# plume-sig/zk-nullifier-sig

Measured on AMD Instinct MI355X. Metric: PLUME verifies/sec (secp256k1 V1) at batch=2^20 per GPU, higher is better.
Workload: dtype u32; 1 GPU; BASELINE.json configs[1]/metric: batch 2^20 per GPU, PLUME V1 verify (secp256k1 + SHA-256), 32-byte messages, 1/16 corrupted, inputs resident in HBM; Fp arithmetic on 9x29-bit limbs through chains of v_mad_u64_u32 (32x32+64); items_per_gpu=1048576, parallelism=shard x1, no collective on the data path, world_size=1

## Files before the change

__graft_entry__.py:

```python
import os
import subprocess
import sys
from pathlib import Path

ROOT = Path(__file__).resolve().parent
os.environ.setdefault("HSA_ENABLE_IPC_MODE_LEGACY", "0")
os.environ.setdefault("GPU_MAX_HW_QUEUES", "8")
if str(ROOT) not in sys.path:
    sys.path.insert(0, str(ROOT))


def build() -> None:
    env = dict(os.environ, PYTORCH_ROCM_ARCH="gfx950")
    subprocess.check_call(["make", "-j2", "-C", str(ROOT / "zk-nullifier-sig_amd" / "csrc")], env=env)
    subprocess.check_call(["make", "-C", str(ROOT / "oracle")])
    subprocess.check_call(["make", "-C", str(ROOT / "tests" / "devsim")])
    subprocess.check_call(["make", "-C", str(ROOT / "tests" / "devgpu")])
    import zk_nullifier_sig_amd as plume
    assert plume.library_path().exists()


def smoke() -> None:
    import numpy as np

    import zk_nullifier_sig_amd as plume
    from oracle import plume_oracle as O
    from tests import _oracle_c as OC
    from tests import synth

    eng = plume.Engine(0)
    n = 64
    for ver in (1, 2):
        b = synth.sign_inputs(n)
        got = eng.sign_batch(ver, b["msgs"], b["off"], b["sk"], b["r"])
        want = OC.sign_batch(ver, b["msgs"], b["off"], b["sk"], b["r"], nthreads=4)
        for k in got:
            assert np.array_equal(got[k], want[k]), f"sign v{ver}: {k} differs from the oracle"
        v = synth.corrupt_for_verify(ver, b, got)
        ok = eng.verify_batch(ver, v["msgs"], v["off"], v["pk"], v["nullifier"], v["c"], v["s"], v.get("r_point"), v.get("hashed_to_curve_r"))
        want_ok = OC.verify_batch(ver, v["msgs"], v["off"], v["pk"], v["nullifier"], v["c"], v["s"], v.get("r_point"), v.get("hashed_to_curve_r"), nthreads=4)
        assert np.array_equal(ok, want_ok), f"verify v{ver} differs from the oracle"
        assert list(ok) == [0 if i % 16 == 5 else 1 for i in range(n)]
        nz = (ver, b["msgs"], b["off"], got["pk"], got["nullifier"], got["s"], got["r_point"], got["hashed_to_curve_r"], got["c"])
        assert np.array_equal(eng.verify_non_zk_batch(*nz), OC.verify_non_zk_batch(*nz, nthreads=4)), f"verify_non_zk v{ver} differs from the oracle"

    class Mock:
        def fill_bytes(self, k):
            return bytes.fromhex("93b9323b629f251b8f3fc2dd11f4672c5544e8230d493eceea98a90bda789808")

    sk = plume.SecretKey.from_bytes(bytes.fromhex("519b423d715f8b581f4fa8ee59f4771a5b44c8130b4e3eacca54a56dda72b464"))
    sig = plume.PlumeSignature.sign_v1(sk, b"An example app message string", Mock(), eng)
    assert sig.c.to_bytes().hex() == "c6a7fc2c926ddbaf20731a479fb6566f2daa5514baae5223fe3b32edbce83254"
    assert sig.s.to_bytes().hex() == "e69f027d84cb6fe5f761e333d12e975fb190d163e8ea132d7de0bd6079ba28ca"
    assert sig.verify(eng)
    assert O.verify(1, sig.message, (sig.pk.x, sig.pk.y), (sig.nullifier.x, sig.nullifier.y), sig.c.value, sig.s.value,
                    (sig.v1specific.r_point.x, sig.v1specific.r_point.y), (sig.v1specific.hashed_to_curve_r.x, sig.v1specific.hashed_to_curve_r.y))
    eng.close()
    print("smoke ok:", plume.library_path())


if __name__ == "__main__":
    build() if (len(sys.argv) < 2 or sys.argv[1] == "build") else smoke()
```

zk-nullifier-sig_amd/csrc/plume_capi.hip:

```cpp
#include <hip/hip_runtime.h>

#include <sched.h>

#include <cctype>
#include <condition_variable>
#include <cstdio>
#include <cstdlib>
#include <cstring>
#include <functional>
#include <iterator>
#include <map>
#include <mutex>
#include <cerrno>
#include <sys/random.h>
#include <string>
#include <thread>
#include <tuple>
#include <initializer_list>
#include <algorithm>
#include <atomic>
#include <memory>
#include <vector>

#include "../../include/plume_hip.h"
// ... 672 lines not shown
}

struct RecoverCall {
    RecoverLaunch fn;
    int version, format;
    uint8_t *rpt, *hr, *h, *status;
};

static int verify_device(plume_ctx* ctx, int version, int mode, size_t n, const uint8_t* msgs, const uint64_t* msg_off, size_t msgs_bytes, const uint8_t* pk, const uint8_t* nul,
                         const uint8_t* c, const uint8_t* s, const uint8_t* rpt, const uint8_t* hr, uint8_t* ok, hipStream_t st,
                         const uint8_t* preflags = nullptr, bool continue_timer = false, const uint8_t* rpt33 = nullptr, const uint8_t* hr33 = nullptr,
                         const RecoverCall* rec = nullptr) {
    if (n == 0) return 0;
    if (n > ctx->chunk) return fail(PLUME_ERR_ARG, "n exceeds the chunk size (plume_set_chunk)");
    if (int rc = need_gtab(ctx)) return rc;
    const bool eq1short = verify_eq1_short(ctx, version, mode, n, rpt != nullptr && rpt33 == nullptr);
    if (eq1short) { if (int rc = need_gcomb(ctx)) return rc; }
    const size_t J = eq1short ? 4 : 3;
    if (!continue_timer) { if (int rc = ws_acquire(ctx, st)) return rc; }
    std::unique_ptr<WsHold> hold(continue_timer ? nullptr : new WsHold(ctx, st));
    const std::vector<size_t> cut = sub_batch_bounds(ctx, n);
    const size_t nsub = cut.size() - 1;
    const bool overlapped = nsub > 1;
    if (int rc = verify_workspace(ctx, n, J, cut)) return rc;
    if (overlapped) { if (int rc = pre_events(ctx, nsub)) return rc; if (int rc = pre_stream(ctx)) return rc; }
    StageTimer& t = ctx->timer;
    if (!continue_timer) t.begin(st);
    hipStream_t pre = overlapped ? ctx->pre : st;
    if (overlapped) {
        HIPCHK(hipEventRecord(ctx->pre_begin, st));
        HIPCHK(hipStreamWaitEvent(pre, ctx->pre_begin, 0));
    }
    for (size_t k = 0; k < nsub; k++) {
        const size_t lo = cut[k], cnt = cut[k + 1] - cut[k];
        VerifyArgs a;
        memset(&a, 0, sizeof a);
        a.version = version; a.mode = mode; a.n = (uint32_t)cnt; a.msgs = msgs; a.msg_off = msg_off + lo; a.msgs_bytes = msgs_bytes;
        a.pk = pk + 64 * lo; a.nul = nul + 64 * lo; a.c = c + 32 * lo; a.s = s + 32 * lo; a.rpt = rpt ? rpt + 64 * lo : nullptr; a.hr = hr ? hr + 64 * lo : nullptr; a.ok = ok ? ok + lo : nullptr;
        a.preflags = preflags ? preflags + lo : nullptr; a.rpt33 = rpt33 ? rpt33 + 33 * lo : nullptr; a.hr33 = hr33 ? hr33 + 33 * lo : nullptr;
        a.bases = ctx->bases.as<uint32_t>() + (size_t)PLUME_BASE_WORDS * J * lo; a.jobflags = ctx->jobflags.as<uint8_t>() + J * lo; a.itemflags = ctx->itemflags.as<uint8_t>() + lo;
        a.tab = ctx->tab.as<uint32_t>() + (size_t)PLUME_TAB_WORDS * J * lo; a.res = ctx->res.as<uint32_t>() + (size_t)PLUME_JAC_WORDS * 2 * lo; a.resinf = ctx->resinf.as<uint8_t>() + 2 * lo;
        a.gtab = ctx->fixed->gtab.as<uint32_t>();
        a.redo = ctx->redo.as<uint32_t>() + 2 * lo + k;
        a.digs = ctx->digs.as<int8_t>() + (size_t)PLUME_VDIG_ROWS * lo;
        if (eq1short) {
            a.eq1fall = ctx->eq1fall.as<uint8_t>() + lo; a.eq1k = ctx->eq1k.as<uint32_t>() + 8 * lo; a.gcomb = ctx->fixed->gcomb.as<uint32_t>();
            a.eq1force = ctx->eq1_short == 2 ? 1 : 0;
        }
        if (k == 0) ctx->redo_counters.clear();
        ctx->redo_counters.push_back(2 * lo + k);
        const bool two_roles = cnt <= ctx->ingest_split_max;
        a.msm_pair = (!eq1short && cnt <= ctx->msm_pair_max) ? 1 : 0;
        a.scalars_in_ingest = two_roles && ctx->split_scalars ? 1 : 0;
        launch_verify_ingest(a, pre, two_roles); if (!overlapped) t.stage(a.scalars_in_ingest ? "verify_ingest_h2c+scalars" : "verify_ingest_h2c", st);
        if (!a.scalars_in_ingest) { launch_verify_scalars(a, pre); if (!overlapped) t.stage("verify_scalars", st); }
        table_stage(ctx, a.tab, a.bases, a.jobflags, J * cnt, 3 * cnt, pre); if (!overlapped) t.stage("tables", st);
        if (overlapped) {
            HIPCHK(hipEventRecord(ctx->pre_ready[k], pre));
            HIPCHK(hipStreamWaitEvent(st, ctx->pre_ready[k], 0));
        }
        ctx->last_msm_kernel = verify_msm_kernel_name(a);
        if (k == 0) ctx->last_msm_sampled = false;
        if (t.on && !overlapped && k == 0) {
            if (ctx->clk.ensure(16)) return PLUME_ERR_HIP;
            HIPCHK(hipMemsetAsync(ctx->clk.p, 0, 16, st));
            a.clk = ctx->clk.as<unsigned long long>();
            ctx->last_msm_sampled = true;
        }
        launch_verify_msm(a, st); if (!overlapped) t.stage("verify_msm", st);
        if (version == 2 && mode == PLUME_MODE_VERIFY) { launch_normalize(a.res, a.resinf, 2 * cnt, st); if (!overlapped) t.stage("to_affine", st); }
        if (rec) {
            const size_t P = recover_width(rec->format);
            RecoverArgs ra;
            memset(&ra, 0, sizeof ra);
            ra.version = rec->version; ra.format = rec->format; ra.n = a.n; ra.pk = a.pk; ra.nul = a.nul; ra.c = a.c;
            ra.itemflags = a.itemflags; ra.jobflags = a.jobflags; ra.tab = a.tab; ra.res = a.res; ra.resinf = a.resinf;
            ra.rpt = rec->rpt ? rec->rpt + P * lo : nullptr; ra.hr = rec->hr ? rec->hr + P * lo : nullptr; ra.h = rec->h ? rec->h + P * lo : nullptr;
            ra.status = rec->status ? rec->status + lo : nullptr;
            rec->fn(ra, st); if (!overlapped) t.stage("recover_finalize", st);
        } else {
            launch_verify_finalize(a, st); if (!overlapped) t.stage("verify_finalize", st);
        }
    }
    if (overlapped) t.stage("verify_overlapped", st);
    HIPCHK(hipGetLastError());
    return hold ? hold->release() : 0;
}

static int sign_device(plume_ctx* ctx, int version, size_t n, const uint8_t* msgs, const uint64_t* msg_off, size_t msgs_bytes, const uint8_t* sk, const uint8_t* r,
                       const uint8_t* pk_in, uint8_t* pk, uint8_t* nul, uint8_t* c, uint8_t* s, uint8_t* rpt, uint8_t* hr, uint8_t* status, uint8_t* h_out,
                       hipStream_t st, bool out33 = false, const uint8_t* aux = nullptr, SignNonceLaunch nonce_fn = nullptr) {
    if (n == 0) return 0;
    if (n > ctx->chunk) return fail(PLUME_ERR_ARG, "n exceeds the chunk size (plume_set_chunk)");
    if (int rc = need_sign_tables(ctx)) return rc;
    const bool selfcheck = ctx->sign_selfcheck != 0;
    const SignReleaseLaunch release_fn = selfcheck ? g_sign_release.load() : nullptr;
    if (selfcheck && !release_fn) return fail(PLUME_ERR_ARG, "the signer's self-check is on but its release kernel is not part of this build");
    const bool sc_eq1short = selfcheck && verify_eq1_short(ctx, version, PLUME_MODE_NON_ZK, n, true);
    if (selfcheck) { if (int rc = need_fixed(ctx, true, sc_eq1short, false)) return rc; }
    if (int rc = ws_acquire(ctx, st)) return rc;
    WsHold hold(ctx, st);
    const std::vector<size_t> cut = sub_batch_bounds(ctx, n);
    constexpr size_t kStageBytes = 4 * 64 + 2 * 32 + 2;
    if (selfcheck && (verify_workspace(ctx, n, sc_eq1short ? 4 : 3, cut) || ctx->scstage.ensure(kStageBytes * n) || (ctx->timer.on && ctx->clk.ensure(16)))) return PLUME_ERR_HIP;
    uint8_t* const stg = ctx->scstage.as<uint8_t>();
    uint8_t *const g_pk = stg, *const g_nul = stg + 64 * n, *const g_rpt = stg + 128 * n, *const g_hr = stg + 192 * n, *const g_c = stg + 256 * n, *const g_s = stg + 288 * n,
            *const g_status = stg + 320 * n, *const g_ok = stg + 321 * n;
    struct StageWipe {
        plume_ctx* ctx; size_t bytes; hipStream_t st;
        ~StageWipe() { if (bytes) (void)hipMemsetAsync(ctx->scstage.p, 0, bytes, st); }
    } stage_wipe{ctx, selfcheck ? kStageBytes * n : 0, st};
    uint8_t *const u_pk = pk, *const u_nul = nul, *const u_c = c, *const u_s = s, *const u_rpt = rpt, *const u_hr = hr, *const u_status = status;
    const bool u_out33 = out33;
    if (selfcheck) { pk = g_pk; nul = g_nul; c = g_c; s = g_s; rpt = g_rpt; hr = g_hr; status = g_status; out33 = false; }
    const size_t nsub = cut.size() - 1;
    const bool overlapped = nsub > 1;
    size_t scr_bytes = 0;
    constexpr size_t SK = PLUME_SIGN_K;
    for (size_t k = 0; k < nsub; k++) scr_bytes = std::max(scr_bytes, table_stage_scratch(ctx, SK * (cut[k + 1] - cut[k]), 0));
    if (ctx->bases.ensure((size_t)PLUME_BASE_WORDS * 4 * SK * n) || ctx->jobflags.ensure(SK * n) || ctx->itemflags.ensure(n) || ctx->tab.ensure((size_t)PLUME_TAB_WORDS * 4 * SK * n) ||
        ctx->tabscr.ensure(scr_bytes) ||
// ... 1441 lines not shown
```

zk-nullifier-sig_amd/csrc/plume_ec.h:

```cpp
#pragma once
#include "plume_field.h"

#if !defined(__HIP_DEVICE_COMPILE__) && defined(PLUME_FE_CHECK)
namespace plume { inline unsigned long& fallback_counter() { static unsigned long c = 0; return c; } }
#define PLUME_COUNT_FALLBACK() (++plume::fallback_counter())
#else
#define PLUME_COUNT_FALLBACK() ((void)0)
#endif

namespace plume {

struct jac {
    fe x, y, z;
    uint32_t inf;
};

PLUME_HD fe fe_beta() { return fe_set(0x7AE96A2Bu, 0x657C0710u, 0x6E64479Eu, 0xAC3434E9u, 0x9CF04975u, 0x12F58995u, 0xC1396C28u, 0x719501EEu); }
PLUME_HD fe fe_gx() { return fe_set(0x79BE667Eu, 0xF9DCBBACu, 0x55A06295u, 0xCE870B07u, 0x029BFCDBu, 0x2DCE28D9u, 0x59F2815Bu, 0x16F81798u); }
PLUME_HD fe fe_gy() { return fe_set(0x483ADA77u, 0x26A3C465u, 0x5DA4FBFCu, 0x0E1108A8u, 0xFD17B448u, 0xA6855419u, 0x9C47D08Fu, 0xFB10D4B8u); }

PLUME_HD fe fe_off_x() { return fe_set(0xBE71E685u, 0x6986BD54u, 0xA5797708u, 0x9EF9F753u, 0x1397E48Bu, 0x08AA9EB1u, 0x128983CAu, 0x1D5B099Bu); }
PLUME_HD fe fe_off_y() { return fe_set(0x15AE5773u, 0x1FAF9233u, 0xF016B8C3u, 0x84D627FDu, 0x8CF7C500u, 0x22EAB6A1u, 0x27C3954Bu, 0x8A01ED04u); }
PLUME_HD fe fe_off_c128_x() { return fe_set(0x8141C548u, 0xF0861E56u, 0xAE562CECu, 0x00E54F8Bu, 0x7535C0B1u, 0x943A12D3u, 0x469080E1u, 0xA23EEBF9u); }
PLUME_HD fe fe_off_c128_y() { return fe_set(0xE429892Au, 0x9AB04F55u, 0xF3E86FE7u, 0xE225348Fu, 0xEF934040u, 0xDC585E87u, 0x1A3CC5BEu, 0x78194203u); }
// ... 206 lines not shown
        if (pos + PLUME_GW_BYTES < PLUME_NDIG) {
            PLUME_UNROLL for (int b = 0; b < PLUME_GW_BYTES; b++) dig[(uint32_t)(pos + b) * stride] = (int8_t)(uint8_t)((mag >> (8 * b)) & 0xFF);
            dig[(uint32_t)(pos + PLUME_GW_BYTES) * stride] = sgn;
        } else if (pos + 1 < PLUME_NDIG) {
            dig[(uint32_t)pos * stride] = (int8_t)(uint8_t)(mag & 0xFF);
            dig[(uint32_t)(pos + 1) * stride] = (int8_t)(uint8_t)(((mag >> 8) & 0x7F) | (sgn ? 0x80 : 0));
        } else {
            dig[(uint32_t)pos * stride] = (int8_t)(uint8_t)((mag & 0x3F) | (sgn ? 0x40 : 0));
        }
    }
}
#define PLUME_NPOS 65
#define PLUME_NPOS64 33
#define PLUME_NPOS66 34
#ifndef PLUME_SIGN_K
#define PLUME_SIGN_K 2
#endif
#define PLUME_SIGN_BITS (128 / PLUME_SIGN_K)
#define PLUME_NPOSK (PLUME_SIGN_BITS / 2 + 1)
static_assert(PLUME_SIGN_K == 2 || PLUME_SIGN_K == 4, "pieces of 64 or 32 bits (whole words of the GLV halves)");
PLUME_HD uint32_t eisd_entry_table(int ta, int tb) {
    static const uint16_t T[64] = {0x240, 0x343, 0x44F, 0x144, 0x261, 0x366, 0x469, 0x167, 0x28D, 0x38C, 0x492, 0x10B, 0x222, 0x328, 0x02A, 0x125,
                                   0x240, 0x343, 0x44F, 0x144, 0x261, 0x366, 0x469, 0x167, 0x28D, 0x38C, 0x011, 0x10B, 0x222, 0x328, 0x02A, 0x125,
                                   0x240, 0x343, 0x44F, 0x144, 0x261, 0x366, 0x469, 0x167, 0x28D, 0x38C, 0x011, 0x10B, 0x222, 0x328, 0x02A, 0x125,
                                   0x240, 0x343, 0x44F, 0x144, 0x261, 0x366, 0x469, 0x167, 0x28D, 0x38C, 0x011, 0x10B, 0x222, 0x328, 0x02A, 0x125};
    const uint32_t idx = (((uint32_t)ta & 3u) << 2) | ((uint32_t)tb & 3u) | (ta < 0 ? 16u : 0u) | (tb < 0 ? 32u : 0u);
    return T[idx];
}
PLUME_HD uint32_t eisd_entry(int ta, int tb) {
    const uint32_t i = (((uint32_t)ta & 3u) << 2) | ((uint32_t)tb & 3u);
    const uint64_t CLO = 0x5C98D3A4C123C60ull, CHI = 0x2A902ull, D0 = 0x2491246DB492ull, D1 = 0x21A31A31A31Aull;
    uint32_t code = (uint32_t)((i < 12u ? CLO >> (5u * i) : CHI >> (5u * (i - 12u))) & 31u);
    uint32_t d0 = (uint32_t)(D0 >> (3u * i)) & 7u, d1 = (uint32_t)(D1 >> (3u * i)) & 7u;
    if (i == 10u && (ta < 0 || tb < 0)) { code = 17u; d0 = 0u; d1 = 0u; }
    return code | (d0 << 5) | (d1 << 8);
}
template <int NP, int NW>
PLUME_HD bool eisd_store(int8_t* dig, uint32_t stride, const uint32_t (&am)[NW], bool aneg, const uint32_t (&bm)[NW], bool bneg, bool flip) {
    const int sa = (aneg != flip) ? -1 : 1, sb = (bneg != flip) ? -1 : 1;
    int ca = 0, cb = 0;
    PLUME_UNROLL for (int i = 0; i < NP; i++) {
        const int w = (2 * i) >> 5, sh = (2 * i) & 31;
        const int cha = w < NW ? (int)((am[w < NW ? w : 0] >> sh) & 3u) : 0, chb = w < NW ? (int)((bm[w < NW ? w : 0] >> sh) & 3u) : 0;
        const int ta = sa * cha + ca, tb = sb * chb + cb;
        const uint32_t e = eisd_entry(ta, tb);
        dig[(uint32_t)i * stride] = (int8_t)(e & 31u);
        ca = (ta - ((int)((e >> 5) & 7u) - 2)) >> 2;
        cb = (tb - ((int)((e >> 8) & 7u) - 2)) >> 2;
    }
    return ca == 0 && cb == 0;
}
PLUME_HD void eisd_store_glv(int8_t* dig, uint32_t stride, const glv_half& h1, const glv_half& h2, bool flip) {
    (void)eisd_store<PLUME_NPOS, 4>(dig, stride, h1.m, h1.neg != 0, h2.m, h2.neg != 0, flip);
}

#define PLUME_TAB_ENTRIES 3
#define PLUME_FE_W PLUME_FE_WORDS
#define PLUME_JAC_WORDS (3 * PLUME_FE_WORDS)
#define PLUME_TAB_ENTRY_WORDS 32
#define PLUME_TAB_WORDS (PLUME_TAB_ENTRIES * PLUME_TAB_ENTRY_WORDS)

PLUME_HD void ld_tab_xy(fe& x, fe& y, const uint32_t* e, bool lambda_half) {
    const uint32_t* xs = lambda_half ? e + 16 : e;
    PLUME_UNROLL for (int i = 0; i < 8; i++) { x.v[i] = xs[i]; y.v[i] = e[8 + i]; }
    x.v[8] = lambda_half ? e[26] : e[24];
    y.v[8] = e[25];
}
template <int ROWS>
PLUME_HD void ld_tab_xy_scan(fe& x, fe& y, const uint32_t* tab, int ad, bool lambda_half) {
    ld_tab_xy(x, y, tab, lambda_half);
    PLUME_NOUNROLL for (int e = 1; e < ROWS; e++) {
        fe rx, ry;
        ld_tab_xy(rx, ry, tab + (size_t)e * PLUME_TAB_ENTRY_WORDS, lambda_half);
        const bool take = ad == e + 1;
        fe_cmov(x, rx, take); fe_cmov(y, ry, take);
    }
}
PLUME_HD void st_tab_entry(uint32_t* e, const fe& x, const fe& y, const fe& bx) {
    PLUME_UNROLL for (int i = 0; i < 8; i++) { e[i] = x.v[i]; e[8 + i] = y.v[i]; e[16 + i] = bx.v[i]; }
    e[24] = x.v[8]; e[25] = y.v[8]; e[26] = bx.v[8]; e[27] = 0;
    e[28] = 0; e[29] = 0; e[30] = 0; e[31] = 0;
}
PLUME_HD void ld_fe(fe& r, const uint32_t* p) { PLUME_UNROLL for (int i = 0; i < PLUME_FE_W; i++) r.v[i] = p[i]; }
PLUME_HD void st_fe(uint32_t* p, const fe& a) { PLUME_UNROLL for (int i = 0; i < PLUME_FE_W; i++) p[i] = a.v[i]; }
PLUME_HD void ld_fe_soa(fe& r, const uint32_t* base, size_t stride, size_t j) { PLUME_UNROLL for (int i = 0; i < PLUME_FE_W; i++) r.v[i] = base[(size_t)i * stride + j]; }
PLUME_HD void st_fe_soa(uint32_t* base, size_t stride, size_t j, const fe& a) { PLUME_UNROLL for (int i = 0; i < PLUME_FE_W; i++) base[(size_t)i * stride + j] = a.v[i]; }
PLUME_HD void ld_jac_soa(jac& p, const uint32_t* base, size_t stride, size_t j) {
    ld_fe_soa(p.x, base, stride, j); ld_fe_soa(p.y, base + PLUME_FE_W * stride, stride, j); ld_fe_soa(p.z, base + 2 * PLUME_FE_W * stride, stride, j);
}
PLUME_HD void st_jac_soa(uint32_t* base, size_t stride, size_t j, const jac& p) {
    st_fe_soa(base, stride, j, p.x); st_fe_soa(base + PLUME_FE_W * stride, stride, j, p.y); st_fe_soa(base + 2 * PLUME_FE_W * stride, stride, j, p.z);
}
#define PLUME_BASE_WORDS 28
struct alignas(16) quad32 { uint32_t a, b, c, d; };
PLUME_HD void st_base(uint32_t* bases, size_t job, const jac& p) {
    quad32* q = reinterpret_cast<quad32*>(bases + job * PLUME_BASE_WORDS);
    q[0] = quad32{p.x.v[0], p.x.v[1], p.x.v[2], p.x.v[3]}; q[1] = quad32{p.x.v[4], p.x.v[5], p.x.v[6], p.x.v[7]};
    q[2] = quad32{p.x.v[8], p.y.v[0], p.y.v[1], p.y.v[2]}; q[3] = quad32{p.y.v[3], p.y.v[4], p.y.v[5], p.y.v[6]};
    q[4] = quad32{p.y.v[7], p.y.v[8], p.z.v[0], p.z.v[1]}; q[5] = quad32{p.z.v[2], p.z.v[3], p.z.v[4], p.z.v[5]};
    q[6] = quad32{p.z.v[6], p.z.v[7], p.z.v[8], 0u};
}
PLUME_HD void ld_base(jac& p, const uint32_t* bases, size_t job, bool with_z) {
    const quad32* q = reinterpret_cast<const quad32*>(bases + job * PLUME_BASE_WORDS);
    const quad32 q0 = q[0], q1 = q[1], q2 = q[2], q3 = q[3], q4 = q[4];
    p.x.v[0] = q0.a; p.x.v[1] = q0.b; p.x.v[2] = q0.c; p.x.v[3] = q0.d; p.x.v[4] = q1.a; p.x.v[5] = q1.b; p.x.v[6] = q1.c; p.x.v[7] = q1.d; p.x.v[8] = q2.a;
    p.y.v[0] = q2.b; p.y.v[1] = q2.c; p.y.v[2] = q2.d; p.y.v[3] = q3.a; p.y.v[4] = q3.b; p.y.v[5] = q3.c; p.y.v[6] = q3.d; p.y.v[7] = q4.a; p.y.v[8] = q4.b;
// ... 458 lines not shown
```

zk-nullifier-sig_amd/csrc/plume_eis.h:

```cpp
#pragma once
#include "plume_ec.h"

namespace plume {

constexpr int kEisR = 5, kEisT = 3;
constexpr int32_t kEisMask = (1 << 29) - 1;

PLUME_HD double eis_fma(double a, double b, double c) { return __builtin_fma(a, b, c); }
template <int N>
PLUME_HD double eis_to_double(const int32_t (&l)[N]) {
    double d = (double)l[N - 1];
    PLUME_UNROLL for (int i = N - 2; i >= 0; i--) d = eis_fma(d, 536870912.0, (double)l[i]);
    return d;
}
template <int N>
PLUME_HD void eis_reduce(int32_t (&x0)[N], int32_t (&x1)[N], const int32_t (&y0)[N], const int32_t (&y1)[N], int32_t q0, int32_t q1) {
    int64_t c0 = 0, c1 = 0;
    PLUME_UNROLL for (int i = 0; i < N; i++) {
        const int32_t z = y0[i] - y1[i];
        c0 += (int64_t)x0[i] - (int64_t)q0 * y0[i] + (int64_t)q1 * y1[i];
        c1 += (int64_t)x1[i] - (int64_t)q0 * y1[i] - (int64_t)q1 * z;
        if (i < N - 1) { x0[i] = (int32_t)c0 & kEisMask; c0 >>= 29; x1[i] = (int32_t)c1 & kEisMask; c1 >>= 29; }
        else { x0[i] = (int32_t)c0; x1[i] = (int32_t)c1; }
    }
// ... 43 lines not shown
    PLUME_UNROLL for (int i = 0; i < N; i++) { x0[i] = x.c0[i]; x1[i] = x.c1[i]; }
}

struct eis_short {
    uint32_t t[2][3], u[2][3];
    uint32_t tneg[2], uneg[2];
    sc tau;
    bool ok;
};
template <int N>
PLUME_HD void eis_from_half(int32_t (&l)[N], const glv_half& h) {
    const uint32_t* m = h.m;
    int32_t v[5];
    v[0] = (int32_t)(m[0] & (uint32_t)kEisMask);
    v[1] = (int32_t)(((m[0] >> 29) | (m[1] << 3)) & (uint32_t)kEisMask);
    v[2] = (int32_t)(((m[1] >> 26) | (m[2] << 6)) & (uint32_t)kEisMask);
    v[3] = (int32_t)(((m[2] >> 23) | (m[3] << 9)) & (uint32_t)kEisMask);
    v[4] = (int32_t)(m[3] >> 20);
    int32_t cy = 0;
    PLUME_UNROLL for (int i = 0; i < N; i++) {
        const int32_t t = (h.neg ? -(i < 5 ? v[i] : 0) : (i < 5 ? v[i] : 0)) + cy;
        if (i < N - 1) { l[i] = t & kEisMask; cy = t >> 29; } else l[i] = t;
    }
}
template <int N>
PLUME_HD bool eis_abs66(uint32_t (&mag)[3], uint32_t& neg, const int32_t (&l)[N]) {
    neg = l[N - 1] < 0 ? 1u : 0u;
    int32_t v[N];
    int32_t cy = 0;
    PLUME_UNROLL for (int i = 0; i < N; i++) {
        const int32_t t = (neg ? -l[i] : l[i]) + cy;
        if (i < N - 1) { v[i] = t & kEisMask; cy = t >> 29; } else v[i] = t;
    }
    const uint32_t a = (uint32_t)v[0], b = (uint32_t)v[1], c = (uint32_t)v[2], d = N > 3 ? (uint32_t)v[N > 3 ? 3 : 0] : 0u;
    mag[0] = a | (b << 29);
    mag[1] = (b >> 3) | (c << 26);
    mag[2] = (c >> 6) | (d << 23);
    bool small = (mag[2] >> 2) == 0 && (N <= 3 || (d >> 9) == 0);
    PLUME_UNROLL for (int i = 4; i < N; i++) small = small && v[i] == 0;
    return small;
}

constexpr int kEisMaxSteps = 400;
PLUME_HD void eis_half_gcd(eis_short& out, const glv_half& g0, const glv_half& g1) {
    const glv_half pa = {{0x9284EB15u, 0xE86C90E4u, 0xA7D46BCDu, 0x3086D221u}, 0u}, pb = {{0x0ABFE4C3u, 0x6F547FA9u, 0x010E8828u, 0xE4437ED6u}, 1u};
    int32_t x0[kEisR], x1[kEisR], y0[kEisR], y1[kEisR];
    eis_from_half(x0, pa); eis_from_half(x1, pb);
    eis_from_half(y0, g0); eis_from_half(y1, g1);
    int32_t tx0[kEisT] = {0, 0, 0}, tx1[kEisT] = {0, 0, 0}, ty0[kEisT] = {1, 0, 0}, ty1[kEisT] = {0, 0, 0};
    double dx0 = eis_to_double(x0), dx1 = eis_to_double(x1), dy0 = eis_to_double(y0), dy1 = eis_to_double(y1);
    const double T = 340282366920938463463374607431768211456.0;
    int which = -1;
    PLUME_NOUNROLL for (int it = 0; it < kEisMaxSteps; it++) {
        if (eis_norm(dy0, dy1) < T) { which = 1; break; }
        int32_t q0, q1; int k;
        eis_quotient(q0, q1, k, dx0, dx1, dy0, dy1);
        eis_step(x0, x1, y0, y1, q0, q1, k);
        eis_step(tx0, tx1, ty0, ty1, q0, q1, k);
        dx0 = eis_to_double(x0); dx1 = eis_to_double(x1);
        if (eis_norm(dx0, dx1) < T) { which = 0; break; }
        eis_quotient(q0, q1, k, dy0, dy1, dx0, dx1);
        eis_step(y0, y1, x0, x1, q0, q1, k);
        eis_step(ty0, ty1, tx0, tx1, q0, q1, k);
        dy0 = eis_to_double(y0); dy1 = eis_to_double(y1);
    }
    const bool sel = which == 1;
    int32_t r0[kEisR], r1[kEisR], t0[kEisT], t1[kEisT];
    PLUME_UNROLL for (int i = 0; i < kEisR; i++) { r0[i] = sel ? y0[i] : x0[i]; r1[i] = sel ? y1[i] : x1[i]; }
    PLUME_UNROLL for (int i = 0; i < kEisT; i++) { t0[i] = sel ? ty0[i] : tx0[i]; t1[i] = sel ? ty1[i] : tx1[i]; }
    bool ok = which >= 0;
    uint32_t m0[3], m1[3], n0, n1;
    ok = eis_abs66(m0, n0, t0) && ok;
    ok = eis_abs66(m1, n1, t1) && ok;
    {
        sc a, b, lam, bl;
        PLUME_UNROLL for (int i = 0; i < 8; i++) { a.v[i] = i < 3 ? m0[i] : 0u; b.v[i] = i < 3 ? m1[i] : 0u; }
        const uint32_t L[8] = {0x1B23BD72u, 0xDF02967Cu, 0x20816678u, 0x122E22EAu, 0x8812645Au, 0xA5261C02u, 0xC05C30E0u, 0x5363AD4Cu};
        PLUME_UNROLL for (int i = 0; i < 8; i++) lam.v[i] = L[i];
        sc_mul(bl, b, lam);
        if (n1) sc_neg(bl, bl);
        if (n0) sc_neg(a, a);
        sc_add(out.tau, a, bl);
        ok = ok && !sc_is_zero(out.tau);
    }
    {
        t0[0] -= 1;
        int32_t cy = 0;
        PLUME_UNROLL for (int i = 0; i < kEisT; i++) { const int32_t t = t0[i] + cy; if (i < kEisT - 1) { t0[i] = t & kEisMask; cy = t >> 29; } else t0[i] = t; }
    }
    ok = eis_abs66(out.t[0], out.tneg[0], t0) && ok;
    PLUME_UNROLL for (int i = 0; i < 3; i++) out.t[1][i] = m1[i];
    out.tneg[1] = n1;
    ok = eis_abs66(out.u[0], out.uneg[0], r0) && ok;
    ok = eis_abs66(out.u[1], out.uneg[1], r1) && ok;
    out.ok = ok;
}

PLUME_HD bool eis_consistent(const eis_short& e, const sc& c) {
    const uint32_t L[8] = {0x1B23BD72u, 0xDF02967Cu, 0x20816678u, 0x122E22EAu, 0x8812645Au, 0xA5261C02u, 0xC05C30E0u, 0x5363AD4Cu};
    sc a, b, lam, bl, ups, lhs;
    PLUME_UNROLL for (int i = 0; i < 8; i++) { a.v[i] = i < 3 ? e.u[0][i] : 0u; b.v[i] = i < 3 ? e.u[1][i] : 0u; lam.v[i] = L[i]; }
    sc_mul(bl, b, lam);
    if (e.uneg[1]) sc_neg(bl, bl);
    if (e.uneg[0]) sc_neg(a, a);
    sc_add(ups, a, bl);
    sc_mul(lhs, e.tau, c);
    uint32_t d = 0;
    PLUME_UNROLL for (int i = 0; i < 8; i++) d |= lhs.v[i] ^ ups.v[i];
    return d == 0;
}

}
```

zk-nullifier-sig_amd/csrc/plume_kernels.hip:

```cpp
#include <algorithm>

#include "plume_launch.h"
#include "plume_dedup.h"

#define PLUME_MIN_WAVES 4
#define PLUME_MSM_WAVES PLUME_MIN_WAVES
#define PLUME_H2C_WAVES 3
#define PLUME_FINAL_WAVES 2
#define PLUME_NORM_WAVES 2
#define PLUME_BOUNDS __launch_bounds__(kBlock, PLUME_MIN_WAVES)
#define PLUME_FINAL_BOUNDS __launch_bounds__(kBlock, PLUME_FINAL_WAVES)
#define PLUME_NORM_BOUNDS __launch_bounds__(kBlock, PLUME_NORM_WAVES)
#define PLUME_MSM_BOUNDS __launch_bounds__(kBlock, PLUME_MSM_WAVES)
#define PLUME_H2C_BOUNDS __launch_bounds__(kBlock, PLUME_H2C_WAVES)

namespace plume {



__global__ PLUME_BOUNDS void k_fixed_bases(uint32_t* base18, uint32_t nwin, uint32_t W) {
    const uint32_t w = blockIdx.x * kBlock + threadIdx.x;
    if (w < nwin) fixed_window_base(base18 + (size_t)w * 2 * PLUME_FE_W, W * w);
}
__global__ PLUME_BOUNDS void k_fixed_table(uint32_t* rows, const uint32_t* base18, uint32_t entries, uint32_t nwin) {
    const size_t lane = (size_t)blockIdx.x * kBlock + threadIdx.x;
    if (lane < (size_t)entries * nwin) fixed_table_lane(rows, base18, entries, lane);
}

__global__ __launch_bounds__(kBlock, 4) void k_verify_scalars(VerifyArgs a) {
    const uint32_t i = blockIdx.x * kBlock + threadIdx.x;
    if (i == 0) a.redo[0] = 0;
    if (i < a.n) verify_scalars(a, i);
}

__global__ PLUME_H2C_BOUNDS void k_verify_ingest(VerifyArgs a) {
    uint32_t i = blockIdx.x * kBlock + threadIdx.x;
    if (i < a.n) verify_ingest_h2c(a, i);
}

__global__ PLUME_H2C_BOUNDS void k_verify_ingest_split(VerifyArgs a) {
    constexpr uint32_t H = kBlock / 2;
    __shared__ uint32_t s_u1[PLUME_FE_WORDS * H];
    __shared__ uint32_t s_q[3 * PLUME_FE_WORDS * H];
    __shared__ uint32_t s_fb[H];
    const uint32_t l = threadIdx.x & (H - 1);
    const bool roleB = threadIdx.x >= H;
    const uint32_t i = blockIdx.x * H + l;
    const bool live = i < a.n;
    if (a.scalars_in_ingest && blockIdx.x == 0 && threadIdx.x == H) a.redo[0] = 0;
    ingest_xch x;
    ingest_a_state st;
    if (live) {
        if (roleB) { verify_ingest_b1(a, i, x); s_fb[l] = x.fb; }
        else { verify_ingest_a1(a, i, x, st); PLUME_UNROLL for (int k = 0; k < PLUME_FE_WORDS; k++) s_u1[k * H + l] = x.u1.v[k]; }
    }
    __syncthreads();
    if (live) {
        if (roleB) {
            PLUME_UNROLL for (int k = 0; k < PLUME_FE_WORDS; k++) x.u1.v[k] = s_u1[k * H + l];
            verify_ingest_b2(x);
            PLUME_UNROLL for (int k = 0; k < PLUME_FE_WORDS; k++) { s_q[k * H + l] = x.xn.v[k]; s_q[(PLUME_FE_WORDS + k) * H + l] = x.xd.v[k]; s_q[(2 * PLUME_FE_WORDS + k) * H + l] = x.y.v[k]; }
        } else {
            x.fb = s_fb[l];
            verify_ingest_a2(a, i, x, st);
        }
    }
    __syncthreads();
    if (live && !roleB) {
        PLUME_UNROLL for (int k = 0; k < PLUME_FE_WORDS; k++) { x.xn.v[k] = s_q[k * H + l]; x.xd.v[k] = s_q[(PLUME_FE_WORDS + k) * H + l]; x.y.v[k] = s_q[(2 * PLUME_FE_WORDS + k) * H + l]; }
        verify_ingest_a3(a, i, x, st);
    } else if (live && a.scalars_in_ingest) {
        verify_scalars(a, i);
    }
}

struct WaveRowSink {
    uint4* rows;
    uint32_t** ptrs;
    bool full;
    __device__ void sync() const { __builtin_amdgcn_fence(__ATOMIC_ACQ_REL, "wavefront"); __builtin_amdgcn_wave_barrier(); }
    __device__ void operator()(uint32_t* e, const fe& x, const fe& y, const fe& bx) const {
        if (!full) { st_tab_entry(e, x, y, bx); return; }
        const uint32_t lane = threadIdx.x & 63u, sw = lane & 7u;
        uint4* mine = rows + lane * 8;
        mine[0 ^ sw] = make_uint4(x.v[0], x.v[1], x.v[2], x.v[3]);
        mine[1 ^ sw] = make_uint4(x.v[4], x.v[5], x.v[6], x.v[7]);
        mine[2 ^ sw] = make_uint4(y.v[0], y.v[1], y.v[2], y.v[3]);
        mine[3 ^ sw] = make_uint4(y.v[4], y.v[5], y.v[6], y.v[7]);
        mine[4 ^ sw] = make_uint4(bx.v[0], bx.v[1], bx.v[2], bx.v[3]);
        mine[5 ^ sw] = make_uint4(bx.v[4], bx.v[5], bx.v[6], bx.v[7]);
        mine[6 ^ sw] = make_uint4(x.v[8], y.v[8], bx.v[8], 0u);
        mine[7 ^ sw] = make_uint4(0u, 0u, 0u, 0u);
        ptrs[lane] = e;
        __builtin_amdgcn_fence(__ATOMIC_RELEASE, "wavefront");
        __builtin_amdgcn_wave_barrier();
        __builtin_amdgcn_fence(__ATOMIC_ACQUIRE, "wavefront");
        const uint32_t quad = lane & 7u;
        PLUME_UNROLL for (uint32_t q = 0; q < 8; q++) {
            const uint32_t r = (lane >> 3) + 8u * q;
            const uint4 v = rows[r * 8 + (quad ^ (r & 7u))];
            reinterpret_cast<uint4*>(ptrs[r])[quad] = v;
        }
        __builtin_amdgcn_fence(__ATOMIC_RELEASE, "wavefront");
        __builtin_amdgcn_wave_barrier();
    }
};

#define PLUME_TABPASS_WAVES_A 4
#define PLUME_TABPASS_WAVES_B 3
#define PLUME_TABINV_K 8
constexpr int kTabBlock = 128;
__global__ __launch_bounds__(kTabBlock, PLUME_TABPASS_WAVES_A) void k_tab_pass_a(const uint32_t* bases, const uint8_t* jobflags, size_t njobs, int L, uint32_t* scr, uint32_t* carry, uint8_t* guardf) {
    const size_t lane = (size_t)blockIdx.x * kTabBlock + threadIdx.x, nl = (size_t)gridDim.x * kTabBlock;
    const size_t j0 = lane * (size_t)L;
    const int cnt = j0 < njobs ? (int)((njobs - j0) < (size_t)L ? (njobs - j0) : (size_t)L) : 0;
    uint32_t* myscr = scr + (size_t)blockIdx.x * ((size_t)L * PLUME_TAB_SCR_WORDS * kTabBlock);
    fe c;
    bool g = false;
    tab_pass_a(bases, jobflags, njobs, j0, cnt, myscr, (size_t)kTabBlock, threadIdx.x, c, g);
    st_fe_soa(carry, nl, lane, c); guardf[lane] = g ? 1 : 0;
}
__global__ __launch_bounds__(kTabBlock, PLUME_TABPASS_WAVES_B) void k_tab_pass_b(uint32_t* tab, const uint32_t* bases, const uint8_t* jobflags, size_t njobs, int L, const uint32_t* scr, const uint32_t* carry,
                                                                                  const uint8_t* guardf) {
    __shared__ uint4 s_rows[kTabBlock * 8];
    __shared__ uint32_t* s_ptrs[kTabBlock];
// ... 370 lines not shown
```

zk-nullifier-sig_amd/csrc/plume_stages.h:

```cpp
#pragma once
#include "plume_h2c.h"
#include "plume_eis.h"

namespace plume {

PLUME_HD uint32_t load_affine_be(fe& x, fe& y, const uint8_t* p) {
    uint32_t wx[8], wy[8];
    words_from_be_aligned(wx, p);
    words_from_be_aligned(wy, p + 32);
    fe_from_words(x, wx);
    fe_from_words(y, wy);
    uint32_t nz = 0;
    PLUME_UNROLL for (int i = 0; i < 8; i++) nz |= wx[i] | wy[i];
    if (nz == 0) return PLUME_JOB_INF;
    if (!words_lt_p(wx) || !words_lt_p(wy)) return PLUME_JOB_INVALID;
    return affine_on_curve(x, y) ? PLUME_JOB_OK : PLUME_JOB_INVALID;
}
PLUME_HD uint32_t reload_affine_be(fe& x, fe& y, const uint8_t* p) {
    uint32_t wx[8], wy[8];
    words_from_be_aligned(wx, p);
    words_from_be_aligned(wy, p + 32);
    fe_from_words(x, wx);
    fe_from_words(y, wy);
    uint32_t nz = 0;
// ... 75 lines not shown
    const bool ok = o1 >= o0 && o1 <= msgs_bytes && o1 - o0 <= 0xFFFFFF00ull;
    len = ok ? (uint32_t)(o1 - o0) : 0u;
    if (!ok) o0 = 0;
    return ok;
}

#define PLUME_MODE_VERIFY 0
#define PLUME_MODE_NON_ZK 1
#define PLUME_ITEM_REJECT 1u
#define PLUME_ITEM_ERR 2u
struct VerifyArgs {
    int version;
    int mode;
    uint32_t n;
    const uint8_t* msgs; const uint64_t* msg_off;
    uint64_t msgs_bytes;
    const uint8_t *pk, *nul, *c, *s, *rpt, *hr;
    uint8_t* ok;
    const uint8_t* preflags;
    const uint8_t *rpt33, *hr33;
    uint32_t* bases;
    uint8_t* jobflags;
    uint8_t* itemflags;
    uint32_t* tab;
    uint32_t* res;
    uint8_t* resinf;
    const uint32_t* gtab;
    uint32_t* redo;
    int8_t* digs;
    uint8_t* eq1fall;
    uint32_t* eq1k;
    const uint32_t* gcomb;
    int msm_pair;
    int scalars_in_ingest;
    unsigned long long* clk;
    int eq1force;
};
PLUME_HD bool verify_eq1_short(const VerifyArgs& a) { return a.eq1fall != nullptr; }
PLUME_HD size_t verify_njobs(const VerifyArgs& a) { return (verify_eq1_short(a) ? 4 : 3) * (size_t)a.n; }
#define PLUME_VDIG_SET PLUME_NPOS
#define PLUME_VDIG_SETB (2 * PLUME_NPOS66)
#define PLUME_VDIG_ROWS (2 * PLUME_VDIG_SET + PLUME_VDIG_SETB)
static_assert(PLUME_VDIG_SETB >= 2 * PLUME_NDIG, "set B holds either form");
PLUME_HD uint32_t redo_file(uint32_t* redo, uint32_t task) {
#if defined(__HIP_DEVICE_COMPILE__)
    const uint32_t k = atomicAdd(redo, 1u);
#else
    const uint32_t k = redo[0]++;
#endif
    redo[1 + k] = task;
    return k;
}

PLUME_HD void verify_item_digits(int8_t* d, uint32_t n, const sc& s, const glv_half& c1, const glv_half& c2, bool long_b) {
    glv_half h1, h2;
    glv_split(h1, h2, s);
    eisd_store_glv(d, n, h1, h2, false);
    if (long_b) { booth_store_wide(d + (size_t)PLUME_VDIG_SET * n, n, h1, false); booth_store_wide(d + (size_t)(PLUME_VDIG_SET + PLUME_NDIG) * n, n, h2, false); }
    eisd_store_glv(d + (size_t)(PLUME_VDIG_SET + PLUME_VDIG_SETB) * n, n, c1, c2, true);
}
PLUME_HD void verify_scalars(const VerifyArgs& a, uint32_t i) {
    sc c, s;
    bool okc = load_scalar_be(c, a.c + 32 * (size_t)i), oks = load_scalar_be(s, a.s + 32 * (size_t)i);
    if (a.mode == PLUME_MODE_NON_ZK) { okc = sc_lt_n(c); oks = sc_lt_n(s); }
    if (!okc || !oks) { if (verify_eq1_short(a)) a.eq1fall[i] = 1; return; }
    bool lng = true;
    glv_half c1, c2;
    glv_split(c1, c2, c);
    if (verify_eq1_short(a)) {
        eis_short e;
        eis_half_gcd(e, c1, c2);
        lng = !e.ok || a.eq1force != 0 || !eis_consistent(e, c);
        if (!lng) {
            sc k;
            sc_mul(k, e.tau, s);
            PLUME_UNROLL for (int w = 0; w < 8; w++) a.eq1k[(size_t)w * a.n + i] = k.v[w];
            int8_t* b = a.digs + (size_t)PLUME_VDIG_SET * a.n + i;
            (void)eisd_store<PLUME_NPOS66, 3>(b, a.n, e.u[0], e.uneg[0] != 0, e.u[1], e.uneg[1] != 0, true);
            (void)eisd_store<PLUME_NPOS66, 3>(b + (size_t)PLUME_NPOS66 * a.n, a.n, e.t[0], e.tneg[0] != 0, e.t[1], e.tneg[1] != 0, true);
        }
        a.eq1fall[i] = lng ? 1 : 0;
    }
    verify_item_digits(a.digs + i, a.n, s, c1, c2, lng);
}

PLUME_HD void verify_ingest_h2c(const VerifyArgs& a, uint32_t i) {
    fe pkx, pky, nx, ny;
    uint32_t fpk = load_affine_be(pkx, pky, a.pk + 64 * (size_t)i);
    uint32_t fnul = load_affine_be(nx, ny, a.nul + 64 * (size_t)i);
    sc c, s;
    bool okc = load_scalar_be(c, a.c + 32 * (size_t)i), oks = load_scalar_be(s, a.s + 32 * (size_t)i);
    if (a.mode == PLUME_MODE_NON_ZK) { okc = sc_lt_n(c); oks = sc_lt_n(s); }
    uint64_t o0; uint32_t mlen;
    const bool okm = msg_span(o0, mlen, a.msg_off, i, a.msgs_bytes);
    bool bad = !okc || !oks || !okm || fpk == PLUME_JOB_INVALID || fnul == PLUME_JOB_INVALID || (a.preflags && a.preflags[i]);
    const bool err = a.mode == PLUME_MODE_NON_ZK && !bad && fpk == PLUME_JOB_INF;
    a.itemflags[i] = (uint8_t)(bad ? PLUME_ITEM_REJECT : err ? PLUME_ITEM_ERR : 0u);
    bad = bad || err;
    if (verify_eq1_short(a)) {
        fe rx, ry;
        const uint32_t fr = load_affine_be(rx, ry, a.rpt + 64 * (size_t)i);
        if (fr == PLUME_JOB_INVALID && !err) { bad = true; a.itemflags[i] = (uint8_t)PLUME_ITEM_REJECT; }
        jac p; p.inf = 0; p.z = fe_small(1); p.x = rx; p.y = ry;
        st_base(a.bases, 3 * (size_t)a.n + i, p); a.jobflags[3 * (size_t)a.n + i] = (uint8_t)(fr | PLUME_JOB_AFFINE);
    }
    {
        jac p; p.inf = 0; p.z = fe_small(1);
        p.x = nx; p.y = ny;
        st_base(a.bases, 3 * (size_t)i + 2, p); a.jobflags[3 * (size_t)i + 2] = (uint8_t)(fnul | PLUME_JOB_AFFINE);
        p.x = pkx; p.y = pky;
        st_base(a.bases, 3 * (size_t)i + 0, p); a.jobflags[3 * (size_t)i + 0] = (uint8_t)(fpk | PLUME_JOB_AFFINE);
    }
    const uint32_t pktag = 2u + (fe_is_odd(pky) ? 1u : 0u);
    jac h;
    if (!bad) {
        hash_to_curve_jac(h, a.msgs + o0, mlen, pkx, pktag, fpk == PLUME_JOB_INF ? PLUME_ENC_IDENTITY : PLUME_ENC_POINT);
    } else {
        h.x = fe_gx(); h.y = fe_gy(); h.z = fe_small(1); h.inf = 0;
    }
    st_base(a.bases, 3 * (size_t)i + 1, h); a.jobflags[3 * (size_t)i + 1] = (uint8_t)(h.inf ? PLUME_JOB_INF : PLUME_JOB_OK);
}

struct ingest_xch {
    fe u1;
    uint32_t fb;
    fe xn, xd, y;
};
struct ingest_a_state { fe u0; fe c, d, y1; uint32_t fpk; bool bad_a, bad; };
PLUME_HD void verify_ingest_b1(const VerifyArgs& a, uint32_t i, ingest_xch& x) {
    fe nx, ny;
    const uint32_t fnul = load_affine_be(nx, ny, a.nul + 64 * (size_t)i);
    sc c, s;
    bool okc = load_scalar_be(c, a.c + 32 * (size_t)i), oks = load_scalar_be(s, a.s + 32 * (size_t)i);
    if (a.mode == PLUME_MODE_NON_ZK) { okc = sc_lt_n(c); oks = sc_lt_n(s); }
    jac p; p.inf = 0; p.z = fe_small(1); p.x = nx; p.y = ny;
    st_base(a.bases, 3 * (size_t)i + 2, p); a.jobflags[3 * (size_t)i + 2] = (uint8_t)(fnul | PLUME_JOB_AFFINE);
    bool okr = true;
// ... 559 lines not shown
```

Baseline: 57.12 million verifies/s.

## Use shared-memory LUT state machine for Eisenstein digit recoding in scalar stage

Replaces the per-digit arithmetic recoding in eisd_store with a 576-word shared-memory lookup table. The table encodes the digit output plus the next carry state, and two digit streams are interleaved per loop so their lookups overlap. The Eisenstein half-GCD loop is restructured to use predicated halves with a single exit test, which cuts divergent branching. The clock-buffer memset is folded into the scalar kernels in place of a separate hipMemsetAsync. In exchange, each block spends time filling the LUT and needs a barrier before use.

```diff
diff --git a/__graft_entry__.py b/__graft_entry__.py
--- a/__graft_entry__.py
+++ b/__graft_entry__.py
@@ -16,6 +16,7 @@
     subprocess.check_call(["make", "-C", str(ROOT / "oracle")])
     subprocess.check_call(["make", "-C", str(ROOT / "tests" / "devsim")])
     subprocess.check_call(["make", "-C", str(ROOT / "tests" / "devgpu")])
+    subprocess.check_call(["make", "-C", str(ROOT / "tests" / "scalar_stage")])
     import zk_nullifier_sig_amd as plume
     assert plume.library_path().exists()
 
diff --git a/zk-nullifier-sig_amd/csrc/plume_capi.hip b/zk-nullifier-sig_amd/csrc/plume_capi.hip
--- a/zk-nullifier-sig_amd/csrc/plume_capi.hip
+++ b/zk-nullifier-sig_amd/csrc/plume_capi.hip
@@ -748,6 +748,12 @@
         const bool two_roles = cnt <= ctx->ingest_split_max;
         a.msm_pair = (!eq1short && cnt <= ctx->msm_pair_max) ? 1 : 0;
         a.scalars_in_ingest = two_roles && ctx->split_scalars ? 1 : 0;
+        if (k == 0) ctx->last_msm_sampled = false;
+        if (t.on && !overlapped && k == 0) {
+            if (ctx->clk.ensure(16)) return PLUME_ERR_HIP;
+            a.clk = ctx->clk.as<unsigned long long>();
+            ctx->last_msm_sampled = true;
+        }
         launch_verify_ingest(a, pre, two_roles); if (!overlapped) t.stage(a.scalars_in_ingest ? "verify_ingest_h2c+scalars" : "verify_ingest_h2c", st);
         if (!a.scalars_in_ingest) { launch_verify_scalars(a, pre); if (!overlapped) t.stage("verify_scalars", st); }
         table_stage(ctx, a.tab, a.bases, a.jobflags, J * cnt, 3 * cnt, pre); if (!overlapped) t.stage("tables", st);
@@ -756,13 +762,6 @@
             HIPCHK(hipStreamWaitEvent(st, ctx->pre_ready[k], 0));
         }
         ctx->last_msm_kernel = verify_msm_kernel_name(a);
-        if (k == 0) ctx->last_msm_sampled = false;
-        if (t.on && !overlapped && k == 0) {
-            if (ctx->clk.ensure(16)) return PLUME_ERR_HIP;
-            HIPCHK(hipMemsetAsync(ctx->clk.p, 0, 16, st));
-            a.clk = ctx->clk.as<unsigned long long>();
-            ctx->last_msm_sampled = true;
-        }
         launch_verify_msm(a, st); if (!overlapped) t.stage("verify_msm", st);
         if (version == 2 && mode == PLUME_MODE_VERIFY) { launch_normalize(a.res, a.resinf, 2 * cnt, st); if (!overlapped) t.stage("to_affine", st); }
         if (rec) {
diff --git a/zk-nullifier-sig_amd/csrc/plume_ec.h b/zk-nullifier-sig_amd/csrc/plume_ec.h
--- a/zk-nullifier-sig_amd/csrc/plume_ec.h
+++ b/zk-nullifier-sig_amd/csrc/plume_ec.h
@@ -282,6 +282,40 @@
 }
 PLUME_HD void eisd_store_glv(int8_t* dig, uint32_t stride, const glv_half& h1, const glv_half& h2, bool flip) {
     (void)eisd_store<PLUME_NPOS, 4>(dig, stride, h1.m, h1.neg != 0, h2.m, h2.neg != 0, flip);
+}
+#define PLUME_EISD_LUT_ROWS 36
+#define PLUME_EISD_LUT_WORDS (PLUME_EISD_LUT_ROWS * 16)
+PLUME_HD uint32_t eisd_lut_word(uint32_t idx) {
+    const uint32_t q = idx / 144u, st = (idx >> 4) % 9u, in = idx & 15u;
+    const int sa = (q & 1u) ? -1 : 1, sb = (q & 2u) ? -1 : 1;
+    const int ca = (int)(st / 3u) - 1, cb = (int)(st % 3u) - 1;
+    const int ta = sa * (int)(in & 3u) + ca, tb = sb * (int)(in >> 2) + cb;
+    const uint32_t e = eisd_entry(ta, tb);
+    const int na = (ta - ((int)((e >> 5) & 7u) - 2)) >> 2, nb = (tb - ((int)((e >> 8) & 7u) - 2)) >> 2;
+    return (e & 31u) | ((q * 9u + (uint32_t)(3 * (na + 1) + (nb + 1))) * 64u) << 8;
+}
+PLUME_HD void eisd_lut_fill(uint32_t* lut, uint32_t tid, uint32_t nthreads) {
+    for (uint32_t k = tid; k < PLUME_EISD_LUT_WORDS; k += nthreads) lut[k] = eisd_lut_word(k);
+}
+template <int NP, int NW>
+PLUME_HD void eisd_store2_lut(const uint32_t* lut, uint32_t stride,
+                              int8_t* dig0, const uint32_t (&am0)[NW], bool aneg0, const uint32_t (&bm0)[NW], bool bneg0, bool flip0,
+                              int8_t* dig1, const uint32_t (&am1)[NW], bool aneg1, const uint32_t (&bm1)[NW], bool bneg1, bool flip1) {
+    const uint32_t q0 = ((aneg0 != flip0) ? 1u : 0u) | ((bneg0 != flip0) ? 2u : 0u), q1 = ((aneg1 != flip1) ? 1u : 0u) | ((bneg1 != flip1) ? 2u : 0u);
+    uint32_t row0 = (q0 * 9u + 4u) * 64u, row1 = (q1 * 9u + 4u) * 64u;
+    const unsigned char* base = reinterpret_cast<const unsigned char*>(lut);
+    PLUME_UNROLL for (int i = 0; i < NP; i++) {
+        const int w = (2 * i) >> 5, sh = (2 * i) & 31;
+        uint32_t in0 = 0u, in1 = 0u;
+        if (w < NW) {
+            in0 = ((am0[w < NW ? w : 0] >> sh) & 3u) | (((bm0[w < NW ? w : 0] >> sh) & 3u) << 2);
+            in1 = ((am1[w < NW ? w : 0] >> sh) & 3u) | (((bm1[w < NW ? w : 0] >> sh) & 3u) << 2);
+        }
+        const uint32_t e0 = *reinterpret_cast<const uint32_t*>(base + (row0 + 4u * in0)), e1 = *reinterpret_cast<const uint32_t*>(base + (row1 + 4u * in1));
+        dig0[(uint32_t)i * stride] = (int8_t)(uint8_t)e0;
+        dig1[(uint32_t)i * stride] = (int8_t)(uint8_t)e1;
+        row0 = e0 >> 8; row1 = e1 >> 8;
+    }
 }
 
 #define PLUME_TAB_ENTRIES 3
diff --git a/zk-nullifier-sig_amd/csrc/plume_eis.h b/zk-nullifier-sig_amd/csrc/plume_eis.h
--- a/zk-nullifier-sig_amd/csrc/plume_eis.h
+++ b/zk-nullifier-sig_amd/csrc/plume_eis.h
@@ -119,17 +119,23 @@
     const double T = 340282366920938463463374607431768211456.0;
     int which = -1;
     PLUME_NOUNROLL for (int it = 0; it < kEisMaxSteps; it++) {
-        if (eis_norm(dy0, dy1) < T) { which = 1; break; }
-        int32_t q0, q1; int k;
-        eis_quotient(q0, q1, k, dx0, dx1, dy0, dy1);
-        eis_step(x0, x1, y0, y1, q0, q1, k);
-        eis_step(tx0, tx1, ty0, ty1, q0, q1, k);
-        dx0 = eis_to_double(x0); dx1 = eis_to_double(x1);
-        if (eis_norm(dx0, dx1) < T) { which = 0; break; }
-        eis_quotient(q0, q1, k, dy0, dy1, dx0, dx1);
-        eis_step(y0, y1, x0, x1, q0, q1, k);
-        eis_step(ty0, ty1, tx0, tx1, q0, q1, k);
-        dy0 = eis_to_double(y0); dy1 = eis_to_double(y1);
+        const bool go_x = !(eis_norm(dy0, dy1) < T);
+        if (go_x) {
+            int32_t q0, q1; int k;
+            eis_quotient(q0, q1, k, dx0, dx1, dy0, dy1);
+            eis_step(x0, x1, y0, y1, q0, q1, k);
+            eis_step(tx0, tx1, ty0, ty1, q0, q1, k);
+            dx0 = eis_to_double(x0); dx1 = eis_to_double(x1);
+        }
+        const bool go_y = go_x && !(eis_norm(dx0, dx1) < T);
+        if (go_y) {
+            int32_t q0, q1; int k;
+            eis_quotient(q0, q1, k, dy0, dy1, dx0, dx1);
+            eis_step(y0, y1, x0, x1, q0, q1, k);
+            eis_step(ty0, ty1, tx0, tx1, q0, q1, k);
+            dy0 = eis_to_double(y0); dy1 = eis_to_double(y1);
+        }
+        if (!go_y) { which = go_x ? 0 : 1; break; }
     }
     const bool sel = which == 1;
     int32_t r0[kEisR], r1[kEisR], t0[kEisT], t1[kEisT];
diff --git a/zk-nullifier-sig_amd/csrc/plume_kernels.hip b/zk-nullifier-sig_amd/csrc/plume_kernels.hip
--- a/zk-nullifier-sig_amd/csrc/plume_kernels.hip
+++ b/zk-nullifier-sig_amd/csrc/plume_kernels.hip
@@ -28,9 +28,15 @@
 }
 
 __global__ __launch_bounds__(kBlock, 4) void k_verify_scalars(VerifyArgs a) {
+    __shared__ uint32_t s_lut[PLUME_EISD_LUT_WORDS];
     const uint32_t i = blockIdx.x * kBlock + threadIdx.x;
-    if (i == 0) a.redo[0] = 0;
-    if (i < a.n) verify_scalars(a, i);
+    if (i == 0) {
+        a.redo[0] = 0;
+        if (a.clk) { a.clk[0] = 0; a.clk[1] = 0; }
+    }
+    eisd_lut_fill(s_lut, threadIdx.x, kBlock);
+    __syncthreads();
+    if (i < a.n) verify_scalars(a, i, s_lut);
 }
 
 __global__ PLUME_H2C_BOUNDS void k_verify_ingest(VerifyArgs a) {
@@ -43,11 +49,16 @@
     __shared__ uint32_t s_u1[PLUME_FE_WORDS * H];
     __shared__ uint32_t s_q[3 * PLUME_FE_WORDS * H];
     __shared__ uint32_t s_fb[H];
+    __shared__ uint32_t s_lut[PLUME_EISD_LUT_WORDS];
     const uint32_t l = threadIdx.x & (H - 1);
     const bool roleB = threadIdx.x >= H;
     const uint32_t i = blockIdx.x * H + l;
     const bool live = i < a.n;
-    if (a.scalars_in_ingest && blockIdx.x == 0 && threadIdx.x == H) a.redo[0] = 0;
+    if (a.scalars_in_ingest && blockIdx.x == 0 && threadIdx.x == H) {
+        a.redo[0] = 0;
+        if (a.clk) { a.clk[0] = 0; a.clk[1] = 0; }
+    }
+    if (a.scalars_in_ingest && roleB) eisd_lut_fill(s_lut, l, H);
     ingest_xch x;
     ingest_a_state st;
     if (live) {
@@ -70,7 +81,7 @@
         PLUME_UNROLL for (int k = 0; k < PLUME_FE_WORDS; k++) { x.xn.v[k] = s_q[k * H + l]; x.xd.v[k] = s_q[(PLUME_FE_WORDS + k) * H + l]; x.y.v[k] = s_q[(2 * PLUME_FE_WORDS + k) * H + l]; }
         verify_ingest_a3(a, i, x, st);
     } else if (live && a.scalars_in_ingest) {
-        verify_scalars(a, i);
+        verify_scalars(a, i, s_lut);
     }
 }
 
diff --git a/zk-nullifier-sig_amd/csrc/plume_stages.h b/zk-nullifier-sig_amd/csrc/plume_stages.h
--- a/zk-nullifier-sig_amd/csrc/plume_stages.h
+++ b/zk-nullifier-sig_amd/csrc/plume_stages.h
@@ -151,14 +151,14 @@
     return k;
 }
 
-PLUME_HD void verify_item_digits(int8_t* d, uint32_t n, const sc& s, const glv_half& c1, const glv_half& c2, bool long_b) {
+PLUME_HD void verify_item_digits(const uint32_t* lut, int8_t* d, uint32_t n, const sc& s, const glv_half& c1, const glv_half& c2, bool long_b) {
     glv_half h1, h2;
     glv_split(h1, h2, s);
-    eisd_store_glv(d, n, h1, h2, false);
+    eisd_store2_lut<PLUME_NPOS, 4>(lut, n, d, h1.m, h1.neg != 0, h2.m, h2.neg != 0, false,
+                                   d + (size_t)(PLUME_VDIG_SET + PLUME_VDIG_SETB) * n, c1.m, c1.neg != 0, c2.m, c2.neg != 0, true);
     if (long_b) { booth_store_wide(d + (size_t)PLUME_VDIG_SET * n, n, h1, false); booth_store_wide(d + (size_t)(PLUME_VDIG_SET + PLUME_NDIG) * n, n, h2, false); }
-    eisd_store_glv(d + (size_t)(PLUME_VDIG_SET + PLUME_VDIG_SETB) * n, n, c1, c2, true);
-}
-PLUME_HD void verify_scalars(const VerifyArgs& a, uint32_t i) {
+}
+PLUME_HD void verify_scalars(const VerifyArgs& a, uint32_t i, const uint32_t* lut) {
     sc c, s;
     bool okc = load_scalar_be(c, a.c + 32 * (size_t)i), oks = load_scalar_be(s, a.s + 32 * (size_t)i);
     if (a.mode == PLUME_MODE_NON_ZK) { okc = sc_lt_n(c); oks = sc_lt_n(s); }
@@ -175,13 +175,22 @@
             sc_mul(k, e.tau, s);
             PLUME_UNROLL for (int w = 0; w < 8; w++) a.eq1k[(size_t)w * a.n + i] = k.v[w];
             int8_t* b = a.digs + (size_t)PLUME_VDIG_SET * a.n + i;
-            (void)eisd_store<PLUME_NPOS66, 3>(b, a.n, e.u[0], e.uneg[0] != 0, e.u[1], e.uneg[1] != 0, true);
-            (void)eisd_store<PLUME_NPOS66, 3>(b + (size_t)PLUME_NPOS66 * a.n, a.n, e.t[0], e.tneg[0] != 0, e.t[1], e.tneg[1] != 0, true);
+            eisd_store2_lut<PLUME_NPOS66, 3>(lut, a.n, b, e.u[0], e.uneg[0] != 0, e.u[1], e.uneg[1] != 0, true,
+                                             b + (size_t)PLUME_NPOS66 * a.n, e.t[0], e.tneg[0] != 0, e.t[1], e.tneg[1] != 0, true);
         }
         a.eq1fall[i] = lng ? 1 : 0;
     }
-    verify_item_digits(a.digs + i, a.n, s, c1, c2, lng);
-}
+    verify_item_digits(lut, a.digs + i, a.n, s, c1, c2, lng);
+}
+#if !defined(__HIP_DEVICE_COMPILE__)
+inline const uint32_t* eisd_lut_host() {
+    struct Lut { uint32_t w[PLUME_EISD_LUT_WORDS]; Lut() { eisd_lut_fill(w, 0u, 1u); } };
+    static const Lut lut;
+    return lut.w;
+}
+inline void verify_scalars(const VerifyArgs& a, uint32_t i) { verify_scalars(a, i, eisd_lut_host()); }
+inline void verify_item_digits(int8_t* d, uint32_t n, const sc& s, const glv_half& c1, const glv_half& c2, bool long_b) { verify_item_digits(eisd_lut_host(), d, n, s, c1, c2, long_b); }
+#endif
 
 PLUME_HD void verify_ingest_h2c(const VerifyArgs& a, uint32_t i) {
     fe pkx, pky, nx, ny;
```

Result: no change. 57.62 million verifies/s, median of 4 (+0.9%).
